# lyclyc52/Instance_NeRF

Measured on AMD Instinct MI355X. Metric: Msamples/sec (train+infer) 3D-FRONT 800x800 at 1/2/4/8 MI355X; PSNR parity, higher is better.
Workload: dtype f32; 1 GPU; render 800x800 synthetic 3D-FRONT-like room, hash-grid NeRF L=16 F=2 T=6119864 sigma+rgb (BASELINE configs[1]), one view per step per GPU; parallelism=views sharded over 1 GPU(s), no data-path collective

## Files before the change

### instance_nerf_amd/build.py

```python
import os
import shutil
import subprocess
import sys

HERE = os.path.dirname(os.path.abspath(__file__))
CSRC = os.path.join(HERE, "csrc")
LIB = os.path.join(CSRC, "libinr_hip.so")
SOURCES = ["raymarch.hip", "encoders.hip", "field_fused.hip", "roialign.hip"]
HEADERS = ["common.h", "grid_common.h", os.path.join("..", "..", "include", "inr.h")]
FLAGS = ["--offload-arch=gfx950", "-O3", "-std=c++17", "-fPIC", "-ffp-contract=off",
         "-munsafe-fp-atomics", "-Wall", "-Wno-unused-function"]


KERNEL_FILES = {
    "field": ["field_fused.hip", "common.h", "grid_common.h"],
    "scatter": ["encoders.hip", "common.h", "grid_common.h"],
}


def source_sha(kind=None):
    import hashlib
    h = hashlib.sha256()
    for f in sorted(KERNEL_FILES[kind] if kind else SOURCES + HEADERS):
        h.update(f.encode())
        h.update(open(os.path.join(CSRC, f), "rb").read())
    return h.hexdigest()


LIB_FP32 = os.path.join(CSRC, "libinr_hip_fp32.so")


def build_fp32(force=False, verbose=True):
    deps = [os.path.join(CSRC, f) for f in SOURCES + HEADERS] + [os.path.abspath(__file__)]
    if not force and os.path.exists(LIB_FP32) and all(os.path.getmtime(d) <= os.path.getmtime(LIB_FP32) for d in deps):
        return LIB_FP32
    hipcc = shutil.which("hipcc") or "/opt/rocm/bin/hipcc"
    objs = []
    for src in SOURCES:
        obj = os.path.join(CSRC, src.replace(".hip", ".fp32.o"))
        cmd = [hipcc, "-x", "hip", "-c", os.path.join(CSRC, src), "-o", obj, "-DINR_MLP_FP32=1"] + FLAGS
        if verbose:
            print(" ".join(cmd), flush=True)
        subprocess.check_call(cmd)
        objs.append(obj)
    subprocess.check_call([hipcc, "-shared", "-o", LIB_FP32] + objs + ["--offload-arch=gfx950"])
    return LIB_FP32


def _stale():
    if not os.path.exists(LIB):
        return True
    t = os.path.getmtime(LIB)
    deps = [os.path.join(CSRC, f) for f in SOURCES + HEADERS] + [os.path.abspath(__file__)]
    return any(os.path.getmtime(d) > t for d in deps)


def build(force=False, verbose=True):
    if not force and not _stale():
        return LIB
    hipcc = shutil.which("hipcc") or "/opt/rocm/bin/hipcc"
    if not os.path.exists(hipcc):
        raise RuntimeError("hipcc not found: cannot build libinr_hip.so")
    objs = []
    for src in SOURCES:
        obj = os.path.join(CSRC, src.replace(".hip", ".o"))
        cmd = [hipcc, "-x", "hip", "-c", os.path.join(CSRC, src), "-o", obj] + FLAGS
        if verbose:
            print(" ".join(cmd), flush=True)
        subprocess.check_call(cmd)
        objs.append(obj)
    cmd = [hipcc, "-shared", "-o", LIB] + objs + ["--offload-arch=gfx950"]
    if verbose:
        print(" ".join(cmd), flush=True)
    subprocess.check_call(cmd)
    return LIB


if __name__ == "__main__":
    build(force="--force" in sys.argv)
    build_fp32(force="--force" in sys.argv)
    print(LIB)
```

### instance_nerf_amd/csrc/field_fused.hip

```cpp
#include <atomic>
#include <mutex>
#include <type_traits>

#include "common.h"
#include "grid_common.h"

namespace inr {

typedef float f32x4 __attribute__((ext_vector_type(4)));
typedef __bf16 bf16x8 __attribute__((ext_vector_type(8)));

#ifndef INR_MLP_FP32
#define INR_MLP_FP32 0
#endif

#ifdef INR_PROBE_BUILD
#include "probe/field_probe.h"
#else
#if defined(INR_PROBE_MODE) || defined(INR_PROBE_STATIC) || defined(INR_PROBE_SLOW_XCD)
#error "INR_PROBE_* switches need -DINR_PROBE_BUILD (tools/build_probe.py): those variants produce wrong results"
#endif
#define INR_PROBE_PROLOGUE()
#define INR_PROBE_SCHEDULE(steal)
#define INR_PROBE_TILE()
#define INR_PROBE_AFTER_GATHER()
#define INR_PROBE_GEO_IS_OUTPUT 1
#define INR_PROBE_EPILOGUE()
#endif


constexpr int kSig0 = 0;
constexpr int kSig1 = kSig0 + 64 * 32;
constexpr int kCol0 = kSig1 + 16 * 64;
constexpr int kCol1 = kCol0 + 64 * 32;
constexpr int kCol2 = kCol1 + 64 * 64;
constexpr int kNerfFloats = kCol2 + 16 * 64;
constexpr int kIns0 = 0;
constexpr int kIns1 = kIns0 + 64 * 32;
constexpr int kIns2 = kIns1 + 64 * 64;

__host__ __device__ inline int frag_pos(int mt, int ks, int lane, int n_ks) {
  return ((mt * (n_ks / 4) + ks / 4) * 64 + lane) * 4 + (ks & 3);
}

__device__ __forceinline__ f32x4 mfma4(const float4 a, const f32x4 b, f32x4 c) {
  c = __builtin_amdgcn_mfma_f32_16x16x4f32(a.x, b[0], c, 0, 0, 0);
  c = __builtin_amdgcn_mfma_f32_16x16x4f32(a.y, b[1], c, 0, 0, 0);
  c = __builtin_amdgcn_mfma_f32_16x16x4f32(a.z, b[2], c, 0, 0, 0);
  c = __builtin_amdgcn_mfma_f32_16x16x4f32(a.w, b[3], c, 0, 0, 0);
  return c;
}
__device__ __forceinline__ float relu1(float x) { return __int_as_float(max(__float_as_int(x), 0)); }
__device__ __forceinline__ f32x4 relu4(f32x4 v) {
  v[0] = relu1(v[0]); v[1] = relu1(v[1]); v[2] = relu1(v[2]); v[3] = relu1(v[3]);
  return v;
}

struct LevelRec {
  uint4 a, b;
};
constexpr int kLevelRecBytes = 16 * sizeof(LevelRec);

__device__ __forceinline__ void stage_level_recs(const GridDesc& G, LevelRec* recs) {
  const int t = threadIdx.x;
  if (t < 16) {
    const int q = t >> 2, li = t & 3;
    const int l = (li >> 1) * 8 + 2 * q + (li & 1);
    const bool live = l < G.num_levels;
    const int lc = live ? l : 0;
    const uint32_t m = G.mask[lc], s = G.res1[lc];
    LevelRec r;
    r.a.x = live ? __float_as_uint(G.scales[lc]) : 0u;
    r.a.y = live ? G.offsets[lc] * 8u : 0u;
    r.a.z = !live ? 0u : (m ? 2654435761u : s);
    r.a.w = !live ? 0u : (m ? 805459861u : s * s);
    r.b.x = !live ? 0u : (m ? m : 0xFFFFFFFFu);
    r.b.y = (live && m) ? 1u : 0u;
    r.b.z = 0u; r.b.w = 0u;
    recs[t] = r;
  }
}

__device__ __forceinline__ bool slot_all_hashed(const GridDesc& G, int li) {
  bool ah = true;
#pragma unroll
  for (int qq = 0; qq < 4; ++qq) {
    const int lq = (li >> 1) * 8 + 2 * qq + (li & 1);
    ah = ah && (lq < G.num_levels) && (G.mask[lq < G.num_levels ? lq : 0] != 0);
  }
  return ah;
}

typedef unsigned int u32x2 __attribute__((__vector_size__(2 * sizeof(unsigned int))));

template <bool kHalf = false>
__device__ __forceinline__ u32x2 gather_row(__amdgpu_buffer_rsrc_t rsrc, uint32_t byte_off) {
  if constexpr (kHalf) {
    u32x2 r;
    r[0] = __builtin_amdgcn_raw_buffer_load_b32(rsrc, (int)(byte_off >> 1), 0, 0);
    r[1] = 0u;
    return r;
  } else {
    return __builtin_amdgcn_raw_buffer_load_b64(rsrc, (int)byte_off, 0, 0);
  }
}

typedef float f32x2 __attribute__((ext_vector_type(2)));

struct Gathered {
  u32x2 c[2][8];
  u32x2 f[4][4];
  float cfx[2], cfy[2], cfz[2];
  float fwx[4], ffy[4], ffz[4];
};

constexpr int kSliceLevels = 3;
constexpr int kWaitAfterCoarse = 8;
constexpr int kWaitBetweenFine = 4;
template <int N>
__device__ __forceinline__ void wait_vmcnt() {
  if constexpr (N >= 0) __builtin_amdgcn_s_waitcnt((N & 0xF) | (0x7 << 4) | (0xF << 8) | ((N >> 4) << 14));
}

template <bool kFineHashed, bool kHalf = false, bool kPre = false>
__device__ __forceinline__ void issue_gathers_impl(const LevelRec* __restrict__ my_recs, __amdgpu_buffer_rsrc_t rsrc,
                                                   float x0, float x1, float x2, Gathered& g) {
  const int q = (threadIdx.x >> 4) & 3;
  const uint32_t side = (uint32_t)(q & 1);
  const LevelRec* pair_recs = my_recs - 4 * (q & 1);
#pragma unroll
  for (int li = 0; li < 2; ++li) {
    const uint4 ra = my_recs[li].a;
    const float s = __uint_as_float(ra.x);
    const uint32_t base = ra.y, pa = ra.z, pb = ra.w;
    const uint32_t mask = my_recs[li].b.x;
    const float px = x0 * s + 0.5f, py = x1 * s + 0.5f, pz = x2 * s + 0.5f;
    g.cfx[li] = __builtin_amdgcn_fractf(px); g.cfy[li] = __builtin_amdgcn_fractf(py); g.cfz[li] = __builtin_amdgcn_fractf(pz);
    const uint32_t cx = (uint32_t)px, cy = (uint32_t)py, cz = (uint32_t)pz;
    const uint32_t hy0 = cy * pa, hy1 = hy0 + pa;
    const uint32_t hz0 = cz * pb, hz1 = hz0 + pb;
    const bool h = my_recs[li].b.y != 0;
    const uint32_t yz[4] = {h ? (hy0 ^ hz0) : (hy0 + hz0), h ? (hy1 ^ hz0) : (hy1 + hz0),
                            h ? (hy0 ^ hz1) : (hy0 + hz1), h ? (hy1 ^ hz1) : (hy1 + hz1)};
#pragma unroll
    for (int k = 0; k < 8; ++k) {
      const uint32_t c = cx + (k & 1);
      const uint32_t idx = (h ? (c ^ yz[k >> 1]) : (c + yz[k >> 1])) & mask;
      g.c[li][k] = gather_row<kHalf>(rsrc, base + idx * 8u);
    }
  }
#pragma unroll
  for (int i = 0; i < 4; ++i) {
    const LevelRec* rec = pair_recs + (i >> 1) * 4 + 2 + (i & 1);
    const uint4 ra = rec->a;
    const float s = __uint_as_float(ra.x);
    const uint32_t base = ra.y, pa = ra.z, pb = ra.w;
    const uint32_t mask = rec->b.x;
    const float px = x0 * s + 0.5f, py = x1 * s + 0.5f, pz = x2 * s + 0.5f;
    const float fx = __builtin_amdgcn_fractf(px);
    g.fwx[i] = side ? fx : 1.0f - fx;
    g.ffy[i] = __builtin_amdgcn_fractf(py); g.ffz[i] = __builtin_amdgcn_fractf(pz);
    const uint32_t c = (uint32_t)px + side, cy = (uint32_t)py, cz = (uint32_t)pz;
    const uint32_t hy0 = cy * pa, hy1 = hy0 + pa;
    const uint32_t hz0 = cz * pb, hz1 = hz0 + pb;
    if (i == 0) wait_vmcnt<kWaitAfterCoarse>();
    else wait_vmcnt<kWaitBetweenFine>();
    if constexpr (kPre) {
      const uint32_t keep = ((q >> 1) && i >= 4 - kSliceLevels) ? 0u : 0xFFFFFFFFu;
      g.f[i][0] = gather_row<kHalf>(rsrc, (base + ((c ^ (hy0 ^ hz0)) & mask) * 8u) & keep);
      g.f[i][1] = gather_row<kHalf>(rsrc, (base + ((c ^ (hy1 ^ hz0)) & mask) * 8u) & keep);
      g.f[i][2] = gather_row<kHalf>(rsrc, (base + ((c ^ (hy0 ^ hz1)) & mask) * 8u) & keep);
      g.f[i][3] = gather_row<kHalf>(rsrc, (base + ((c ^ (hy1 ^ hz1)) & mask) * 8u) & keep);
    } else if constexpr (kFineHashed) {
      g.f[i][0] = gather_row<kHalf>(rsrc, base + ((c ^ (hy0 ^ hz0)) & mask) * 8u);
      g.f[i][1] = gather_row<kHalf>(rsrc, base + ((c ^ (hy1 ^ hz0)) & mask) * 8u);
      g.f[i][2] = gather_row<kHalf>(rsrc, base + ((c ^ (hy0 ^ hz1)) & mask) * 8u);
      g.f[i][3] = gather_row<kHalf>(rsrc, base + ((c ^ (hy1 ^ hz1)) & mask) * 8u);
    } else {
      const bool h = rec->b.y != 0;
      const uint32_t yz[4] = {h ? (hy0 ^ hz0) : (hy0 + hz0), h ? (hy1 ^ hz0) : (hy1 + hz0),
                              h ? (hy0 ^ hz1) : (hy0 + hz1), h ? (hy1 ^ hz1) : (hy1 + hz1)};
#pragma unroll
      for (int k = 0; k < 4; ++k) {
        const uint32_t idx = (h ? (c ^ yz[k]) : (c + yz[k])) & mask;
        g.f[i][k] = gather_row<kHalf>(rsrc, base + idx * 8u);
      }
    }
  }
}

template <bool kHalf = false, bool kPre = false>
__device__ __forceinline__ void issue_gathers(const LevelRec* __restrict__ my_recs, const bool (&all_hashed)[4],
                                              __amdgpu_buffer_rsrc_t rsrc, float x0, float x1, float x2, Gathered& g) {
  if constexpr (kPre) issue_gathers_impl<true, kHalf, true>(my_recs, rsrc, x0, x1, x2, g);
  else if (all_hashed[2] && all_hashed[3]) issue_gathers_impl<true, kHalf>(my_recs, rsrc, x0, x1, x2, g);
  else issue_gathers_impl<false, kHalf>(my_recs, rsrc, x0, x1, x2, g);
}

template <bool kHalf = false>
__device__ __forceinline__ f32x2 row2(const u32x2 v) {
  const unsigned bx = v[0], by = v[1];
  if constexpr (kHalf) {
    typedef _Float16 h2 __attribute__((ext_vector_type(2)));
    const h2 h = __builtin_bit_cast(h2, bx);
    return f32x2{(float)h[0], (float)h[1]};
  } else {
    return f32x2{__uint_as_float(bx), __uint_as_float(by)};
  }
}

template <bool kHalf = false>
__device__ __forceinline__ void blend(const Gathered& g, f32x4& lo, f32x4& hi) {
#pragma unroll
  for (int li = 0; li < 2; ++li) {
    const f32x2 wx = {1.0f - g.cfx[li], g.cfx[li]};
    const float wy0 = 1.0f - g.cfy[li], wz0 = 1.0f - g.cfz[li];
    const f32x2 a = wx * wy0, b = wx * g.cfy[li];
    const f32x2 w[4] = {a * wz0, b * wz0, a * g.cfz[li], b * g.cfz[li]};
    f32x2 acc = {0.f, 0.f};
#pragma unroll
    for (int k = 0; k < 8; ++k) {
      const f32x2 wk = (k & 1) ? w[k >> 1].yy : w[k >> 1].xx;
      acc = __builtin_elementwise_fma(wk, row2<kHalf>(g.c[li][k]), acc);
    }
    lo[2 * li] = acc.x;
    lo[2 * li + 1] = acc.y;
  }
  f32x2 part[4];
#pragma unroll
  for (int i = 0; i < 4; ++i) {
    const f32x2 wy = {1.0f - g.ffy[i], g.ffy[i]};
    const f32x2 xy = wy * g.fwx[i];
    const f32x2 w0 = xy * (1.0f - g.ffz[i]), w1 = xy * g.ffz[i];
    f32x2 acc = {0.f, 0.f};
    acc = __builtin_elementwise_fma(w0.xx, row2<kHalf>(g.f[i][0]), acc);
    acc = __builtin_elementwise_fma(w0.yy, row2<kHalf>(g.f[i][1]), acc);
    acc = __builtin_elementwise_fma(w1.xx, row2<kHalf>(g.f[i][2]), acc);
    acc = __builtin_elementwise_fma(w1.yy, row2<kHalf>(g.f[i][3]), acc);
    part[i] = acc;
  }
#pragma unroll
  for (int t = 0; t < 4; ++t) {
    const int lv = t >> 1, ft = t & 1;
    const auto r = __builtin_amdgcn_permlane16_swap(__float_as_uint(part[lv][ft]), __float_as_uint(part[2 + lv][ft]), false, false);
    const unsigned r0 = r[0], r1 = r[1];
    hi[t] = __uint_as_float(r0) + __uint_as_float(r1);
  }
}


template <int N_MT, int N_G>
__device__ __forceinline__ void layer(const float4* __restrict__ w, int lane, const f32x4* in, f32x4* out) {
  if constexpr (N_MT == 1) {
    f32x4 a0 = {0.f, 0.f, 0.f, 0.f}, a1 = {0.f, 0.f, 0.f, 0.f};
#pragma unroll
    for (int g = 0; g < N_G; g += 2) {
      __builtin_amdgcn_sched_barrier(0);
      const float4 w0 = w[g * 64 + lane], w1 = w[(g + 1) * 64 + lane];
      a0 = __builtin_amdgcn_mfma_f32_16x16x4f32(w0.x, in[g][0], a0, 0, 0, 0);
      a1 = __builtin_amdgcn_mfma_f32_16x16x4f32(w1.x, in[g + 1][0], a1, 0, 0, 0);
      a0 = __builtin_amdgcn_mfma_f32_16x16x4f32(w0.y, in[g][1], a0, 0, 0, 0);
      a1 = __builtin_amdgcn_mfma_f32_16x16x4f32(w1.y, in[g + 1][1], a1, 0, 0, 0);
      a0 = __builtin_amdgcn_mfma_f32_16x16x4f32(w0.z, in[g][2], a0, 0, 0, 0);
      a1 = __builtin_amdgcn_mfma_f32_16x16x4f32(w1.z, in[g + 1][2], a1, 0, 0, 0);
      a0 = __builtin_amdgcn_mfma_f32_16x16x4f32(w0.w, in[g][3], a0, 0, 0, 0);
      a1 = __builtin_amdgcn_mfma_f32_16x16x4f32(w1.w, in[g + 1][3], a1, 0, 0, 0);
    }
    out[0] = a0 + a1;
  } else {
    f32x4 acc[N_MT];
#pragma unroll
    for (int mt = 0; mt < N_MT; ++mt) acc[mt] = f32x4{0.f, 0.f, 0.f, 0.f};
#pragma unroll
    for (int g = 0; g < N_G; ++g) {
      __builtin_amdgcn_sched_barrier(0);
      float4 wv[N_MT];
#pragma unroll
      for (int mt = 0; mt < N_MT; ++mt) wv[mt] = w[(mt * N_G + g) * 64 + lane];
#pragma unroll
      for (int mt = 0; mt < N_MT; ++mt) acc[mt] = __builtin_amdgcn_mfma_f32_16x16x4f32(wv[mt].x, in[g][0], acc[mt], 0, 0, 0);
#pragma unroll
      for (int mt = 0; mt < N_MT; ++mt) acc[mt] = __builtin_amdgcn_mfma_f32_16x16x4f32(wv[mt].y, in[g][1], acc[mt], 0, 0, 0);
#pragma unroll
      for (int mt = 0; mt < N_MT; ++mt) acc[mt] = __builtin_amdgcn_mfma_f32_16x16x4f32(wv[mt].z, in[g][2], acc[mt], 0, 0, 0);
#pragma unroll
      for (int mt = 0; mt < N_MT; ++mt) acc[mt] = __builtin_amdgcn_mfma_f32_16x16x4f32(wv[mt].w, in[g][3], acc[mt], 0, 0, 0);
    }
#pragma unroll
    for (int mt = 0; mt < N_MT; ++mt) out[mt] = acc[mt];
  }
}

struct SplitB {
  uint4 hi, lo;
};

__device__ __forceinline__ void split2(float x0, float x1, uint32_t& hi, uint32_t& lo) {
  const uint32_t u0 = __float_as_uint(x0), u1 = __float_as_uint(x1);
  hi = __builtin_amdgcn_perm(u1, u0, 0x07060302u);
  const float l0 = x0 - __uint_as_float(u0 & 0xFFFF0000u);
  const float l1 = x1 - __uint_as_float(u1 & 0xFFFF0000u);
  lo = __builtin_amdgcn_perm(__float_as_uint(l1), __float_as_uint(l0), 0x07060302u);
}
__device__ __forceinline__ SplitB split8(const f32x4 a, const f32x4 b) {
  SplitB r;
  split2(a[0], a[1], r.hi.x, r.lo.x);
  split2(a[2], a[3], r.hi.y, r.lo.y);
  split2(b[0], b[1], r.hi.z, r.lo.z);
  split2(b[2], b[3], r.hi.w, r.lo.w);
  return r;
}
__device__ __forceinline__ f32x4 mfma_bf(const uint4 a, const uint4 b, const f32x4 c) {
  return __builtin_amdgcn_mfma_f32_16x16x32_bf16(__builtin_bit_cast(bf16x8, a), __builtin_bit_cast(bf16x8, b), c, 0, 0, 0);
}

template <int N_MT, int N_S>
__device__ __forceinline__ void layer_bf(const uint4* __restrict__ w, int lane, const SplitB* in, f32x4* out) {
  if constexpr (N_MT == 1) {
    f32x4 a0 = {0.f, 0.f, 0.f, 0.f}, a1 = a0, a2 = a0;
#pragma unroll
    for (int st = 0; st < N_S; ++st) {
      __builtin_amdgcn_sched_barrier(0);
      const uint4 wh = w[(st * 2 + 0) * 64 + lane], wlo = w[(st * 2 + 1) * 64 + lane];
      a0 = mfma_bf(wh, in[st].hi, a0);
      a1 = mfma_bf(wlo, in[st].hi, a1);
      a2 = mfma_bf(wh, in[st].lo, a2);
    }
    out[0] = a0 + (a1 + a2);
  } else {
    f32x4 acc[N_MT];
#pragma unroll
    for (int mt = 0; mt < N_MT; ++mt) acc[mt] = f32x4{0.f, 0.f, 0.f, 0.f};
#pragma unroll
    for (int st = 0; st < N_S; ++st) {
      __builtin_amdgcn_sched_barrier(0);
      uint4 wh[N_MT], wlo[N_MT];
#pragma unroll
      for (int mt = 0; mt < N_MT; ++mt) {
        wh[mt] = w[((mt * N_S + st) * 2 + 0) * 64 + lane];
        wlo[mt] = w[((mt * N_S + st) * 2 + 1) * 64 + lane];
      }
#pragma unroll
      for (int mt = 0; mt < N_MT; ++mt) acc[mt] = mfma_bf(wh[mt], in[st].hi, acc[mt]);
#pragma unroll
      for (int mt = 0; mt < N_MT; ++mt) acc[mt] = mfma_bf(wlo[mt], in[st].hi, acc[mt]);
#pragma unroll
      for (int mt = 0; mt < N_MT; ++mt) acc[mt] = mfma_bf(wh[mt], in[st].lo, acc[mt]);
    }
#pragma unroll
    for (int mt = 0; mt < N_MT; ++mt) out[mt] = acc[mt];
  }
}

typedef _Float16 f16x8_t __attribute__((ext_vector_type(8)));
typedef _Float16 f16x2_t __attribute__((ext_vector_type(2)));
typedef float f32x2_t __attribute__((ext_vector_type(2)));
__device__ __forceinline__ uint32_t pack_f16x2(float a, float b) {
  const f32x2_t v = {a, b};
  return __builtin_bit_cast(uint32_t, __builtin_convertvector(v, f16x2_t));
}
template <int N_MT, int N_S>
__device__ __forceinline__ void layer_h1(const uint4* __restrict__ w, int lane, const uint4* in, f32x4* out) {
  f32x4 acc[N_MT];
#pragma unroll
  for (int mt = 0; mt < N_MT; ++mt) acc[mt] = f32x4{0.f, 0.f, 0.f, 0.f};
#pragma unroll
  for (int st = 0; st < N_S; ++st) {
    __builtin_amdgcn_sched_barrier(0);
#pragma unroll
    for (int mt = 0; mt < N_MT; ++mt)
      acc[mt] = __builtin_amdgcn_mfma_f32_16x16x32_f16(__builtin_bit_cast(f16x8_t, w[((mt * N_S + st) * 2 + 0) * 64 + lane]),
                                                       __builtin_bit_cast(f16x8_t, in[st]), acc[mt], 0, 0, 0);
  }
#pragma unroll
  for (int mt = 0; mt < N_MT; ++mt) out[mt] = acc[mt];
}

template <int N_MT, int N_G, bool kFast = false>
__device__ __forceinline__ void mlp_layer(const float4* __restrict__ wsec, int lane, const f32x4* in, f32x4* out) {
#if INR_MLP_FP32
  layer<N_MT, N_G>(wsec, lane, in, out);
#else
  if constexpr (kFast) {
    uint4 b[N_G / 2];
#pragma unroll
    for (int st = 0; st < N_G / 2; ++st)
      b[st] = uint4{pack_f16x2(in[2 * st][0], in[2 * st][1]), pack_f16x2(in[2 * st][2], in[2 * st][3]),
                    pack_f16x2(in[2 * st + 1][0], in[2 * st + 1][1]), pack_f16x2(in[2 * st + 1][2], in[2 * st + 1][3])};
    layer_h1<N_MT, N_G / 2>(reinterpret_cast<const uint4*>(wsec), lane, b, out);
  } else {
    SplitB b[N_G / 2];
#pragma unroll
    for (int st = 0; st < N_G / 2; ++st) b[st] = split8(in[2 * st], in[2 * st + 1]);
    layer_bf<N_MT, N_G / 2>(reinterpret_cast<const uint4*>(wsec), lane, b, out);
  }
#endif
}

__device__ __forceinline__ float select4(int q, float a, float b, float c, float d) {
  return q == 0 ? a : (q == 1 ? b : (q == 2 ? c : d));
}

struct TileIn {
  float x0, x1, x2;
  float d0, d1, d2;
  bool oob;
};

__device__ __forceinline__ float to_x01(float x, float bound, float rb, float) { return (x + bound) / rb; }

template <bool kDir>
__device__ __forceinline__ void load_tile_in(const float* __restrict__ x, const float* __restrict__ d, int64_t m,
                                             float bound, float rb, float rb_inv, TileIn& t) {
  t.x0 = to_x01(x[m * 3 + 0], bound, rb, rb_inv);
  t.x1 = to_x01(x[m * 3 + 1], bound, rb, rb_inv);
  t.x2 = to_x01(x[m * 3 + 2], bound, rb, rb_inv);
  t.oob = oob01(t.x0, t.x1, t.x2);
  if (t.oob) t.x0 = t.x1 = t.x2 = 0.0f;
  if constexpr (kDir) {
    t.d0 = d[m * 3]; t.d1 = d[m * 3 + 1]; t.d2 = d[m * 3 + 2];
  }
}

constexpr int kXcdChunkLog2 = 10;
#ifndef INR_STEAL_SHIFT
#define INR_STEAL_SHIFT 1
#endif
constexpr int kStealRoundsShift = INR_STEAL_SHIFT;
struct TileSched {
  int64_t lo, hi;
  int64_t first;
  int64_t stride;
  int64_t main_local = 0, tail_base = 0;
  int64_t n_main = 0, tail = 0;
  int64_t static_local = 0;
  uint32_t xcd = 0;
  bool interleaved = false, hybrid = false;
  __device__ __forceinline__ int64_t tile_of(int y, int64_t u) const {
    if (u < main_local) return ((((u >> kXcdChunkLog2) << 3) + y) << kXcdChunkLog2) + (u & ((1 << kXcdChunkLog2) - 1));
    return n_main + tail * y / 8 + (u - main_local);
  }
  __device__ __forceinline__ int64_t local_end(int y) const { return main_local + tail * (y + 1) / 8 - tail * y / 8; }
  __device__ __forceinline__ int64_t tile(int64_t i) const {
    if (interleaved) {
      const int64_t u = first + i * stride;
      if (u < main_local)
        return ((((u >> kXcdChunkLog2) << 3) + xcd) << kXcdChunkLog2) + (u & ((1 << kXcdChunkLog2) - 1));
      return tail_base + (u - main_local);
    }
    return first + i * stride;
  }
};
__device__ __forceinline__ TileSched make_sched(int64_t n_tiles, int waves_per_block, bool steal = false) {
  const int nb = gridDim.x, b = blockIdx.x;
  const int w = threadIdx.x >> 6;
  TileSched s;
  if (nb % 8 == 0) {
    const int xcd = b & 7, local = b >> 3, per = nb >> 3;
    const int64_t rounds = n_tiles >> (kXcdChunkLog2 + 3);
    if (rounds >= 4) {
      const int64_t n_main = rounds << (kXcdChunkLog2 + 3), tail = n_tiles - n_main;
      s.interleaved = true;
      s.xcd = (uint32_t)xcd;
      s.main_local = rounds << kXcdChunkLog2;
      s.n_main = n_main;
      s.tail = tail;
      s.hybrid = steal;
      s.static_local = steal ? (rounds - max((int64_t)1, rounds >> kStealRoundsShift)) << kXcdChunkLog2 : s.main_local;
      s.tail_base = n_main + tail * xcd / 8;
      s.lo = 0;
      s.hi = n_main + tail * (xcd + 1) / 8;
      s.first = (int64_t)local * waves_per_block + w;
      s.stride = (int64_t)per * waves_per_block;
      return s;
    }
    s.lo = n_tiles * xcd / 8;
    s.hi = n_tiles * (xcd + 1) / 8;
    s.first = s.lo + (int64_t)local * waves_per_block + w;
    s.stride = (int64_t)per * waves_per_block;
  } else {
    s.lo = 0;
    s.hi = n_tiles;
    s.first = (int64_t)b * waves_per_block + w;
    s.stride = (int64_t)nb * waves_per_block;
  }
  return s;
}

constexpr int kFieldThreads = 512;
constexpr int kGroupChunkLog2 = 6;
constexpr int kGroupDraw = 1;
constexpr int kGroupPools = 4;
struct GroupDraw {
  unsigned long long* cursor;
  int owner, n_owner;
  __device__ __forceinline__ void init(unsigned long long* cursors, int pools) {
    const int n_xcd = (gridDim.x % 8 == 0) ? 8 : 1;
    const int n_pool = (gridDim.x % (8 * pools) == 0) ? pools : 1;
    const int xcd = (n_xcd == 8) ? (int)(blockIdx.x & 7) : 0;
    const int pool = (n_pool > 1) ? (int)((blockIdx.x >> 3) % pools) : 0;
    owner = pool * n_xcd + xcd;
    n_owner = n_pool * n_xcd;
    cursor = cursors + owner;
  }
  __device__ __forceinline__ int64_t group_of(uint32_t u) const {
    const int64_t chunk = (int64_t)(u >> kGroupChunkLog2) * n_owner + owner;
    return (chunk << kGroupChunkLog2) + (u & ((1u << kGroupChunkLog2) - 1u));
  }
  __device__ __forceinline__ int64_t draw() const { return group_of((uint32_t)atomicAdd(cursor, (unsigned long long)kGroupDraw)); }
};
constexpr int kStealPools = 4, kStealOwners = 8 * kStealPools, kStealDraw = 4, kStealBlockLog2 = 6;
struct TileWalk {
  TileSched s;
  unsigned long long* cur;
  int lane, own, owner, sub;
  int64_t it, k_base;
  unsigned long long raw_next;
  bool dyn;
  __device__ __forceinline__ void init(const TileSched& sched, unsigned long long* cursors) {
    s = sched; cur = cursors; lane = threadIdx.x & 63; it = 0; dyn = false; sub = kStealDraw; k_base = 0; raw_next = 0;
    own = owner = (int)(((blockIdx.x >> 3) % kStealPools) * 8 + (blockIdx.x & 7));
    if (!cursors) s.hybrid = false;
    if (!s.hybrid) s.static_local = s.main_local;
  }
  __device__ __forceinline__ int64_t pool_len(int o) const {
    const int64_t nb = (s.local_end(o & 7) - s.static_local + (1 << kStealBlockLog2) - 1) >> kStealBlockLog2;
    const int p = o >> 3;
    return nb > p ? ((nb - p + kStealPools - 1) / kStealPools) << kStealBlockLog2 : 0;
  }
  __device__ __forceinline__ int64_t local_of(int o, int64_t k) const {
    return s.static_local + ((((k >> kStealBlockLog2) * kStealPools) + (o >> 3)) << kStealBlockLog2) +
           (k & ((1 << kStealBlockLog2) - 1));
  }
  __device__ __forceinline__ unsigned long long issue(int o) const {
    unsigned long long v = 0;
    if (lane == 0) v = atomicAdd(cur + o, (unsigned long long)kStealDraw);
    return v;
  }
  __device__ __forceinline__ static int64_t uniform(unsigned long long v) {
    return (int64_t)(((unsigned long long)(uint32_t)__builtin_amdgcn_readfirstlane((int)(v >> 32)) << 32) |
                     (uint32_t)__builtin_amdgcn_readfirstlane((int)v));
  }
  __device__ __forceinline__ int scan() const {
    bool live = false;
    if (lane < kStealOwners) live = (int64_t)__hip_atomic_load(cur + lane, __ATOMIC_RELAXED, __HIP_MEMORY_SCOPE_AGENT) < pool_len(lane);
    const uint32_t mask = (uint32_t)__ballot(live);
    for (int i = 0; i < kStealOwners; ++i) {
      const int o = (((own >> 3) + i) % kStealPools) * 8 + (((own & 7) + i / kStealPools) & 7);
      if ((mask >> o) & 1u) return o;
    }
    return -1;
  }
  __device__ __forceinline__ int64_t next() {
    if (!dyn) {
      if (!s.hybrid) {
        const int64_t t = s.tile(it++);
        return t < s.hi ? t : -1;
      }
      const int64_t u = s.first + (it++) * s.stride;
      if (u < s.static_local) return s.tile_of((int)s.xcd, u);
      dyn = true;
      raw_next = issue(owner);
    }
    for (;;) {
      if (sub < kStealDraw) {
        const int64_t u = local_of(owner, k_base + sub);
        ++sub;
        if (u < s.local_end(owner & 7)) return s.tile_of(owner & 7, u);
        continue;
      }
      int64_t k = uniform(raw_next);
      while (k >= pool_len(owner)) {
        const int o = scan();
        if (o < 0) return -1;
        owner = o;
        k = uniform(issue(owner));
      }
      k_base = k;
      sub = 0;
      raw_next = issue(owner);
    }
  }
};
constexpr int kFieldMinWaves = 2;

__device__ __forceinline__ f32x4 load4(const float* p) {
  const float4 v = *reinterpret_cast<const float4*>(p);
  return f32x4{v.x, v.y, v.z, v.w};
}
__device__ __forceinline__ void store4(float* p, f32x4 v) {
  *reinterpret_cast<float4*>(p) = make_float4(v[0], v[1], v[2], v[3]);
}
__device__ __forceinline__ f32x4 mask4(f32x4 g, f32x4 h) {
  return f32x4{h[0] > 0.f ? g[0] : 0.f, h[1] > 0.f ? g[1] : 0.f, h[2] > 0.f ? g[2] : 0.f, h[3] > 0.f ? g[3] : 0.f};
}

struct NerfSave {
  float *enc, *h1, *so, *cin, *c1, *c2;
};

template <bool kColor, bool kTable = false, int kSave = 0, bool kHalf = false, bool kFast = false, bool kPre = false>
__global__ void __launch_bounds__(kFieldThreads, kFieldMinWaves) k_nerf_fwd(const float* __restrict__ x, const float* __restrict__ d,
                                                               int64_t M, const int32_t* __restrict__ n_dev, float bound,
                                                               const float2* __restrict__ emb, uint32_t emb_bytes, GridDesc G,
                                                               const float4* __restrict__ packed, float density_scale,
                                                               float* __restrict__ sigma, float* __restrict__ rgb,
                                                               float* __restrict__ geo, const int32_t* __restrict__ ray_ids,
                                                               const float4* __restrict__ shq, NerfSave sv,
                                                               unsigned long long* __restrict__ steal) {
  extern __shared__ __attribute__((aligned(16))) float4 wl[];
  INR_PROBE_PROLOGUE();
  __builtin_amdgcn_s_setprio(3);
  constexpr int kStage = (kColor ? kNerfFloats : kCol0) / 4;
  for (int i = threadIdx.x; i < kStage; i += kFieldThreads) wl[i] = packed[i];
  LevelRec* recs = reinterpret_cast<LevelRec*>(wl + kStage);
  stage_level_recs(G, recs);
  __syncthreads();

  constexpr int kWaves = kFieldThreads / 64;
  const int lane = threadIdx.x & 63, q = lane >> 4, j = lane & 15;
  int64_t n = M;
  if (n_dev) n = min((int64_t)*n_dev, M);
  const int64_t n_tiles = (n + 15) >> 4;
  const float rb = 2.0f * bound;
  const float rb_inv = 0.0f;
  INR_PROBE_SCHEDULE(steal);
  TileWalk walk;
  walk.init(make_sched(n_tiles, kWaves, steal != nullptr), steal);

  const bool all_hashed[4] = {slot_all_hashed(G, 0), slot_all_hashed(G, 1), slot_all_hashed(G, 2), slot_all_hashed(G, 3)};
  const __amdgpu_buffer_rsrc_t rsrc = __builtin_amdgcn_make_buffer_rsrc((void*)emb, 0, (int)emb_bytes, 0x00020000);

  for (int64_t tile = walk.next(); tile >= 0; tile = walk.next()) {
    INR_PROBE_TILE();
    const int64_t m = tile * 16 + j;
    const bool valid = m < n;
    TileIn me;
    f32x4 sh_in = {0.f, 0.f, 0.f, 0.f};
    if constexpr (kTable) {
      const int64_t mm = valid ? m : n - 1;
      me.x0 = x[mm * 3 + 0]; me.x1 = x[mm * 3 + 1]; me.x2 = x[mm * 3 + 2];
      const float4 t4 = shq[(int64_t)ray_ids[mm] * 4 + q];
      sh_in = f32x4{t4.x, t4.y, t4.z, t4.w};
    } else {
      load_tile_in<kColor>(x, d, valid ? m : n - 1, bound, rb, rb_inv, me);
    }

    f32x4 enc[2];
    {
      Gathered g;
      uint32_t rec_off = (uint32_t)q * 4u * (uint32_t)sizeof(LevelRec);
      asm volatile("" : "+v"(rec_off));
      typedef float v2f __attribute__((ext_vector_type(2)));
      v2f fine_a = {0.f, 0.f}, fine_b = {0.f, 0.f};
      if constexpr (kPre) {
        static_assert(!kPre || kTable, "the sliced feed is a variant of the table feed");
        static_assert(kSliceLevels == 3, "lane map below");
        const v2f* pre = reinterpret_cast<const v2f*>(d);
        const int64_t m_pad = (M + 31) & ~(int64_t)31, mm = valid ? m : n - 1;
        const int sl = (q & 1) ? 1 : 0;
        fine_a = __builtin_nontemporal_load(pre + (int64_t)sl * m_pad + mm);
        fine_b = __builtin_nontemporal_load(pre + (int64_t)(sl + 1) * m_pad + mm);
      }
      issue_gathers<kHalf, kPre>(reinterpret_cast<const LevelRec*>(reinterpret_cast<const char*>(recs) + rec_off), all_hashed,
                                 rsrc, me.x0, me.x1, me.x2, g);
      __builtin_amdgcn_sched_barrier(0);
      blend<kHalf>(g, enc[0], enc[1]);
      if constexpr (kPre) {
        if (q == 2) enc[1] = f32x4{enc[1][0], enc[1][1], fine_a.x, fine_a.y};
        else if (q == 3) enc[1] = f32x4{fine_a.x, fine_a.y, fine_b.x, fine_b.y};
      }
    }
    if constexpr (!kTable) {
      if (me.oob) enc[0] = enc[1] = f32x4{0.f, 0.f, 0.f, 0.f};
    }
    INR_PROBE_AFTER_GATHER();

    f32x4 h1[4];
    mlp_layer<4, 2, kFast>(wl + kSig0 / 4, lane, enc, h1);
#pragma unroll
    for (int t = 0; t < 4; ++t) h1[t] = relu4(h1[t]);
    f32x4 h2[1];
    mlp_layer<1, 4, kFast>(wl + kSig1 / 4, lane, h1, h2);

    if (valid) {
      if (q == 0) sigma[m] = __expf(h2[0][0]) * density_scale;
      if (INR_PROBE_GEO_IS_OUTPUT && geo) {
#pragma unroll
        for (int r = 0; r < 4; ++r) {
          const int row = 4 * q + r;
          if (row >= 1) geo[m * 15 + row - 1] = h2[0][r];
        }
      }
    }

    if constexpr (kColor) {
      f32x4 cin[2];
      if constexpr (kTable) {
        cin[0] = sh_in;
      } else {
        float sh[16];
        sh4(me.d0, me.d1, me.d2, sh);
#pragma unroll
        for (int ks = 0; ks < 4; ++ks) cin[0][ks] = select4(q, sh[4 * ks], sh[4 * ks + 1], sh[4 * ks + 2], sh[4 * ks + 3]);
      }
      cin[1] = h2[0];
      f32x4 c1[4], c2[4], o[1];
      mlp_layer<4, 2, kFast>(wl + kCol0 / 4, lane, cin, c1);
#pragma unroll
      for (int t = 0; t < 4; ++t) c1[t] = relu4(c1[t]);
      mlp_layer<4, 4, kFast>(wl + kCol1 / 4, lane, c1, c2);
#pragma unroll
      for (int t = 0; t < 4; ++t) c2[t] = relu4(c2[t]);
      mlp_layer<1, 4, kFast>(wl + kCol2 / 4, lane, c2, o);
      if constexpr (kSave == 2) {
        if (valid) {
#pragma unroll
          for (int t = 0; t < 2; ++t) store4(sv.enc + m * 32 + 16 * t + 4 * q, enc[t]);
        }
      }
      if constexpr (kSave == 1) {
        if (valid) {
#pragma unroll
          for (int t = 0; t < 2; ++t) store4(sv.enc + m * 32 + 16 * t + 4 * q, enc[t]);
          store4(sv.so + m * 16 + 4 * q, h2[0]);
#pragma unroll
          for (int t = 0; t < 4; ++t) {
            store4(sv.h1 + m * 64 + 16 * t + 4 * q, h1[t]);
            store4(sv.c1 + m * 64 + 16 * t + 4 * q, c1[t]);
            store4(sv.c2 + m * 64 + 16 * t + 4 * q, c2[t]);
          }
#pragma unroll
          for (int ks = 0; ks < 4; ++ks) sv.cin[m * 32 + 4 * ks + q] = cin[0][ks];
#pragma unroll
          for (int r = 0; r < 4; ++r) {
            const int row = 4 * q + r;
            sv.cin[m * 32 + (row >= 1 ? 15 + row : 31)] = row >= 1 ? h2[0][r] : 0.f;
          }
        }
      }
      if (valid && q == 0) {
        rgb[m * 3 + 0] = __frcp_rn(1.0f + __expf(-o[0][0]));
        rgb[m * 3 + 1] = __frcp_rn(1.0f + __expf(-o[0][1]));
        rgb[m * 3 + 2] = __frcp_rn(1.0f + __expf(-o[0][2]));
      }
    }
  }
  INR_PROBE_EPILOGUE();
}

constexpr int kSliceThreads = 256;
constexpr int kSliceTilesPerIter = 4;
struct SliceX {
  float x0, x1, x2;
};
__device__ __forceinline__ SliceX slice_load_x(const float* __restrict__ x01, int64_t m, int64_t M) {
  const int64_t mm = m < M ? m : M - 1;
  const float* p = x01 + mm * 3;
  return SliceX{__builtin_nontemporal_load(p), __builtin_nontemporal_load(p + 1), __builtin_nontemporal_load(p + 2)};
}
__global__ void __launch_bounds__(kSliceThreads) k_grid_fine_slices(const float* __restrict__ x01, int64_t M,
                                                                    const float2* __restrict__ emb, uint32_t emb_bytes,
                                                                    GridDesc G, float* __restrict__ pre) {
  const int slice = blockIdx.y;
  const int l = 16 - kSliceLevels + slice;
  const float sc = G.scales[l];
  const uint32_t m_ = G.mask[l], res1 = G.res1[l];
  const bool h = m_ != 0;
  const uint32_t base = G.offsets[l] * 8u, pa = h ? 2654435761u : res1, pb = h ? 805459861u : res1 * res1;
  const uint32_t mask = h ? m_ : 0xFFFFFFFFu;
  const __amdgpu_buffer_rsrc_t rsrc = __builtin_amdgcn_make_buffer_rsrc((void*)emb, 0, (int)emb_bytes, 0x00020000);
  const int lane = threadIdx.x & 63, w = threadIdx.x >> 6;
  const uint32_t side = (uint32_t)(lane & 1);
  constexpr int kWaves = kSliceThreads / 64;
  constexpr int kT = kSliceTilesPerIter;
  const int64_t m_pad = (M + 31) & ~(int64_t)31;
  const int64_t n_iter = (M + 32 * kT - 1) / (32 * kT);
  float* __restrict__ out = pre + (int64_t)slice * m_pad * 2;
  for (int64_t it = (int64_t)blockIdx.x * kWaves + w; it < n_iter; it += (int64_t)gridDim.x * kWaves) {
    u32x2 rows[kT][4];
    float wx[kT], fy[kT], fz[kT];
#pragma unroll
    for (int t = 0; t < kT; ++t) {
      const SliceX X = slice_load_x(x01, (it * kT + t) * 32 + (lane >> 1), M);
      const float px = X.x0 * sc + 0.5f, py = X.x1 * sc + 0.5f, pz = X.x2 * sc + 0.5f;
      const float fx = __builtin_amdgcn_fractf(px);
      wx[t] = side ? fx : 1.0f - fx;
      fy[t] = __builtin_amdgcn_fractf(py); fz[t] = __builtin_amdgcn_fractf(pz);
      const uint32_t c = (uint32_t)px + side, cy = (uint32_t)py, cz = (uint32_t)pz;
      const uint32_t hy0 = cy * pa, hy1 = hy0 + pa;
      const uint32_t hz0 = cz * pb, hz1 = hz0 + pb;
      const uint32_t yz[4] = {h ? (hy0 ^ hz0) : (hy0 + hz0), h ? (hy1 ^ hz0) : (hy1 + hz0),
                              h ? (hy0 ^ hz1) : (hy0 + hz1), h ? (hy1 ^ hz1) : (hy1 + hz1)};
#pragma unroll
      for (int k = 0; k < 4; ++k) {
        const uint32_t idx = (h ? (c ^ yz[k]) : (c + yz[k])) & mask;
        rows[t][k] = gather_row<false>(rsrc, base + idx * 8u);
      }
    }
#pragma unroll
    for (int t = 0; t < kT; ++t) {
      const f32x2 wy = {1.0f - fy[t], fy[t]};
      const f32x2 xy = wy * wx[t];
      const f32x2 w0 = xy * (1.0f - fz[t]), w1 = xy * fz[t];
      f32x2 acc = {0.f, 0.f};
      acc = __builtin_elementwise_fma(w0.xx, row2<false>(rows[t][0]), acc);
      acc = __builtin_elementwise_fma(w0.yy, row2<false>(rows[t][1]), acc);
      acc = __builtin_elementwise_fma(w1.xx, row2<false>(rows[t][2]), acc);
      acc = __builtin_elementwise_fma(w1.yy, row2<false>(rows[t][3]), acc);
      const float ox = __shfl_xor(acc.x, 1), oy = __shfl_xor(acc.y, 1);
      const float v = side ? acc.y + oy : acc.x + ox;
      const int64_t m = (it * kT + t) * 32 + (lane >> 1);
      if (m < M) __builtin_nontemporal_store(v, out + m * 2 + side);
    }
  }
}

struct LatticeDesc {
  const float* ax_w;
  const float* ax_l;
  const float* ax_h;
  int W, L, H, Wp;
};
constexpr int kMaxExtractDirs = 8;
template <bool kLattice>
__global__ void __launch_bounds__(kFieldThreads, kFieldMinWaves) k_nerf_fwd_dirs(
    const float* __restrict__ x, int64_t M, float bound, const float2* __restrict__ emb, uint32_t emb_bytes, GridDesc G,
    const float4* __restrict__ packed, const float* __restrict__ sh_dirs , int D, float4* __restrict__ out,
    LatticeDesc lat, float logit_min) {
  extern __shared__ __attribute__((aligned(16))) float4 wl[];
  constexpr int kStage = kNerfFloats / 4;
  for (int i = threadIdx.x; i < kStage; i += kFieldThreads) wl[i] = packed[i];
  LevelRec* recs = reinterpret_cast<LevelRec*>(wl + kStage);
  stage_level_recs(G, recs);
  float* shl = reinterpret_cast<float*>(recs + 16);
  for (int i = threadIdx.x; i < D * 16; i += kFieldThreads) {
    const int d = i >> 4, qq = (i >> 2) & 3, ks = i & 3;
    shl[i] = sh_dirs[d * 16 + 4 * ks + qq];
  }
  __syncthreads();
  constexpr int kWaves = kFieldThreads / 64;
  const int lane = threadIdx.x & 63, q = lane >> 4, j = lane & 15;
  const int64_t n_tiles = (M + 15) >> 4;
  const float rb = 2.0f * bound;
  const TileSched sched = make_sched(n_tiles, kWaves);
  const bool all_hashed[4] = {slot_all_hashed(G, 0), slot_all_hashed(G, 1), slot_all_hashed(G, 2), slot_all_hashed(G, 3)};
  const __amdgpu_buffer_rsrc_t rsrc = __builtin_amdgcn_make_buffer_rsrc((void*)emb, 0, (int)emb_bytes, 0x00020000);
  const float inv_d = 1.0f / (float)D;
  for (int64_t it = 0, tile = sched.tile(0); tile < sched.hi; tile = sched.tile(++it)) {
    int64_t m = tile * 16 + j;
    bool valid = m < M;
    TileIn me;
    if constexpr (kLattice) {
      const int64_t row = m / lat.Wp;
      const int iw = (int)(m - row * lat.Wp);
      const int il = (int)(row / lat.H), ih = (int)(row - (int64_t)il * lat.H);
      valid = valid && iw < lat.W;
      const int cw = min(iw, lat.W - 1), cl = min(il, lat.L - 1);
      me.x0 = to_x01(fminf(fmaxf(lat.ax_w[cw], -bound), bound), bound, rb, 0.0f);
      me.x1 = to_x01(fminf(fmaxf(lat.ax_l[cl], -bound), bound), bound, rb, 0.0f);
      me.x2 = to_x01(fminf(fmaxf(lat.ax_h[ih], -bound), bound), bound, rb, 0.0f);
      me.oob = oob01(me.x0, me.x1, me.x2);
      if (me.oob) me.x0 = me.x1 = me.x2 = 0.0f;
      m = ((int64_t)cw * lat.L + cl) * lat.H + ih;
    } else {
      load_tile_in<false>(x, nullptr, valid ? m : M - 1, bound, rb, 0.0f, me);
    }
    f32x4 enc[2];
    {
      Gathered g;
      uint32_t rec_off = (uint32_t)q * 4u * (uint32_t)sizeof(LevelRec);
      asm volatile("" : "+v"(rec_off));
      issue_gathers(reinterpret_cast<const LevelRec*>(reinterpret_cast<const char*>(recs) + rec_off), all_hashed, rsrc,
                    me.x0, me.x1, me.x2, g);
      __builtin_amdgcn_sched_barrier(0);
      blend(g, enc[0], enc[1]);
    }
    if (me.oob) enc[0] = enc[1] = f32x4{0.f, 0.f, 0.f, 0.f};
    f32x4 h1[4], h2[1];
    mlp_layer<4, 2>(wl + kSig0 / 4, lane, enc, h1);
#pragma unroll
    for (int t = 0; t < 4; ++t) h1[t] = relu4(h1[t]);
    mlp_layer<1, 4>(wl + kSig1 / 4, lane, h1, h2);
    float r = 0.f, g = 0.f, b = 0.f;
    for (int d = 0; d < D; ++d) {
      f32x4 cin[2], c1[4], c2[4], o[1];
      const float4 s4 = *reinterpret_cast<const float4*>(shl + d * 16 + q * 4);
      cin[0] = f32x4{s4.x, s4.y, s4.z, s4.w};
      cin[1] = h2[0];
      mlp_layer<4, 2>(wl + kCol0 / 4, lane, cin, c1);
#pragma unroll
      for (int t = 0; t < 4; ++t) c1[t] = relu4(c1[t]);
      mlp_layer<4, 4>(wl + kCol1 / 4, lane, c1, c2);
#pragma unroll
      for (int t = 0; t < 4; ++t) c2[t] = relu4(c2[t]);
      mlp_layer<1, 4>(wl + kCol2 / 4, lane, c2, o);
      r += __frcp_rn(1.0f + __expf(-o[0][0]));
      g += __frcp_rn(1.0f + __expf(-o[0][1]));
      b += __frcp_rn(1.0f + __expf(-o[0][2]));
    }
    if (valid && q == 0) out[m] = make_float4(r * inv_d, g * inv_d, b * inv_d, fmaxf(h2[0][0], logit_min));
  }
}

template <int K_MT, int kSave = 0>
__global__ void __launch_bounds__(kFieldThreads, kFieldMinWaves) k_instance_fwd(const float* __restrict__ x, int64_t M,
                                                                   const int32_t* __restrict__ n_dev, float bound,
                                                                   const float2* __restrict__ emb, uint32_t emb_bytes,
                                                                   GridDesc G, const float4* __restrict__ packed,
                                                                   float* __restrict__ logits, float* __restrict__ enc_out,
                                                                   float* __restrict__ h1_out, float* __restrict__ h2_out) {
  extern __shared__ __attribute__((aligned(16))) float4 wl[];
  constexpr int K = K_MT * 16;
  constexpr int kStage = (kIns2 + K * 64) / 4;
  for (int i = threadIdx.x; i < kStage; i += kFieldThreads) wl[i] = packed[i];
  LevelRec* recs = reinterpret_cast<LevelRec*>(wl + kStage);
  stage_level_recs(G, recs);
  __syncthreads();

  constexpr int kWaves = kFieldThreads / 64;
  const int lane = threadIdx.x & 63, q = lane >> 4, j = lane & 15;
  int64_t n = M;
  if (n_dev) n = min((int64_t)*n_dev, M);
  const int64_t n_tiles = (n + 15) >> 4;
  const float rb = 2.0f * bound;
  const float rb_inv = 0.0f;
  const TileSched sched = make_sched(n_tiles, kWaves);

  const bool all_hashed[4] = {slot_all_hashed(G, 0), slot_all_hashed(G, 1), slot_all_hashed(G, 2), slot_all_hashed(G, 3)};
  const __amdgpu_buffer_rsrc_t rsrc = __builtin_amdgcn_make_buffer_rsrc((void*)emb, 0, (int)emb_bytes, 0x00020000);

  for (int64_t it = 0, tile = sched.tile(0); tile < sched.hi; tile = sched.tile(++it)) {
    const int64_t m = tile * 16 + j;
    const bool valid = m < n;
    TileIn me;
    load_tile_in<false>(x, nullptr, valid ? m : n - 1, bound, rb, rb_inv, me);
    f32x4 enc[2];
    {
      Gathered g;
      uint32_t rec_off = (uint32_t)q * 4u * (uint32_t)sizeof(LevelRec);
      asm volatile("" : "+v"(rec_off));
      issue_gathers(reinterpret_cast<const LevelRec*>(reinterpret_cast<const char*>(recs) + rec_off), all_hashed, rsrc,
                    me.x0, me.x1, me.x2, g);
      __builtin_amdgcn_sched_barrier(0);
      blend(g, enc[0], enc[1]);
    }
    if (me.oob) enc[0] = enc[1] = f32x4{0.f, 0.f, 0.f, 0.f};
    f32x4 h1[4], h2[4], o[K_MT];
    mlp_layer<4, 2>(wl + kIns0 / 4, lane, enc, h1);
#pragma unroll
    for (int t = 0; t < 4; ++t) h1[t] = relu4(h1[t]);
    mlp_layer<4, 4>(wl + kIns1 / 4, lane, h1, h2);
#pragma unroll
    for (int t = 0; t < 4; ++t) h2[t] = relu4(h2[t]);
    mlp_layer<K_MT, 4>(wl + kIns2 / 4, lane, h2, o);
    if (valid) {
#pragma unroll
      for (int mt = 0; mt < K_MT; ++mt) {
        float4 v = make_float4(o[mt][0], o[mt][1], o[mt][2], o[mt][3]);
        *reinterpret_cast<float4*>(logits + m * K + 16 * mt + 4 * q) = v;
      }
      if constexpr (kSave != 0) {
#pragma unroll
        for (int t = 0; t < 2; ++t)
          *reinterpret_cast<float4*>(enc_out + m * 32 + 16 * t + 4 * q) = make_float4(enc[t][0], enc[t][1], enc[t][2], enc[t][3]);
      }
      if constexpr (kSave == 1) {
#pragma unroll
        for (int t = 0; t < 4; ++t) {
          *reinterpret_cast<float4*>(h1_out + m * 64 + 16 * t + 4 * q) = make_float4(h1[t][0], h1[t][1], h1[t][2], h1[t][3]);
          *reinterpret_cast<float4*>(h2_out + m * 64 + 16 * t + 4 * q) = make_float4(h2[t][0], h2[t][1], h2[t][2], h2[t][3]);
        }
      }
    }
  }
}

constexpr uint8_t kLabelEmpty = 255;
constexpr int kNoChannel = 0x7fffffff;
template <int K_MT>
__global__ void __launch_bounds__(kFieldThreads, kFieldMinWaves) k_instance_lattice(
    LatticeDesc lat, float bound, const float2* __restrict__ emb_n, uint32_t emb_n_bytes, GridDesc Gn,
    const float4* __restrict__ packed_n, float density_scale, float sigma_thresh, const float2* __restrict__ emb_i,
    uint32_t emb_i_bytes, GridDesc Gi, const float4* __restrict__ packed_i, int K, uint8_t* __restrict__ labels,
    float* __restrict__ confidence, float* __restrict__ logit_out) {
  extern __shared__ __attribute__((aligned(16))) float4 wl[];
  constexpr int kStageN = kCol0 / 4;
  constexpr int kStageI = (kIns2 + K_MT * 16 * 64) / 4;
  const float4* wn = wl;
  const float4* wi = wl + kStageN;
  for (int i = threadIdx.x; i < kStageN; i += kFieldThreads) wl[i] = packed_n[i];
  for (int i = threadIdx.x; i < kStageI; i += kFieldThreads) wl[kStageN + i] = packed_i[i];
  LevelRec* recs_n = reinterpret_cast<LevelRec*>(wl + kStageN + kStageI);
  LevelRec* recs_i = recs_n + 16;
  stage_level_recs(Gn, recs_n);
  stage_level_recs(Gi, recs_i);
  __syncthreads();

  constexpr int kWaves = kFieldThreads / 64;
  const int lane = threadIdx.x & 63, q = lane >> 4, j = lane & 15;
  const int64_t n_tiles = ((int64_t)lat.Wp * lat.L * lat.H) >> 4;
  const float rb = 2.0f * bound;
  const TileSched sched = make_sched(n_tiles, kWaves);
  const bool hashed_n[4] = {slot_all_hashed(Gn, 0), slot_all_hashed(Gn, 1), slot_all_hashed(Gn, 2), slot_all_hashed(Gn, 3)};
  const bool hashed_i[4] = {slot_all_hashed(Gi, 0), slot_all_hashed(Gi, 1), slot_all_hashed(Gi, 2), slot_all_hashed(Gi, 3)};
  const __amdgpu_buffer_rsrc_t rsrc_n = __builtin_amdgcn_make_buffer_rsrc((void*)emb_n, 0, (int)emb_n_bytes, 0x00020000);
  const __amdgpu_buffer_rsrc_t rsrc_i = __builtin_amdgcn_make_buffer_rsrc((void*)emb_i, 0, (int)emb_i_bytes, 0x00020000);
  for (int64_t it = 0, tile = sched.tile(0); tile < sched.hi; tile = sched.tile(++it)) {
    const int64_t m = tile * 16 + j;
    const int64_t row = m / lat.Wp;
    const int iw = (int)(m - row * lat.Wp);
    const int il = (int)(row / lat.H), ih = (int)(row - (int64_t)il * lat.H);
    const bool valid = iw < lat.W;
    const int cw = min(iw, lat.W - 1);
    TileIn me;
    me.x0 = to_x01(fminf(fmaxf(lat.ax_w[cw], -bound), bound), bound, rb, 0.0f);
    me.x1 = to_x01(fminf(fmaxf(lat.ax_l[il], -bound), bound), bound, rb, 0.0f);
// ... 1818 lines not shown
```

Before: 6474 Msamples/s.

## Software-pipeline split-bf16 MLP layers with interleaved weight prefetch and ReLU splitting

Replaces the per-layer split-bf16 MFMA MLP calls in the sigma and color nets with hand-scheduled chains. These prefetch the next weight fragment one slot ahead and do the ReLU plus hi/lo bf16 split of the previous output tile inside the current tile's MFMA slot, using sched_group_barrier to interleave MFMA and VALU work. The aim is to hide weight-load latency and layer-boundary VALU work behind matrix instructions. The cost is higher register pressure, which may lower occupancy, and more rigid instruction scheduling. The shared split2 helper moves into a new header.

```diff
diff --git a/instance_nerf_amd/build.py b/instance_nerf_amd/build.py
--- a/instance_nerf_amd/build.py
+++ b/instance_nerf_amd/build.py
@@ -7,13 +7,13 @@
 CSRC = os.path.join(HERE, "csrc")
 LIB = os.path.join(CSRC, "libinr_hip.so")
 SOURCES = ["raymarch.hip", "encoders.hip", "field_fused.hip", "roialign.hip"]
-HEADERS = ["common.h", "grid_common.h", os.path.join("..", "..", "include", "inr.h")]
+HEADERS = ["common.h", "grid_common.h", "bf16_split.h", os.path.join("..", "..", "include", "inr.h")]
 FLAGS = ["--offload-arch=gfx950", "-O3", "-std=c++17", "-fPIC", "-ffp-contract=off",
          "-munsafe-fp-atomics", "-Wall", "-Wno-unused-function"]
 
 
 KERNEL_FILES = {
-    "field": ["field_fused.hip", "common.h", "grid_common.h"],
+    "field": ["field_fused.hip", "common.h", "grid_common.h", "bf16_split.h"],
     "scatter": ["encoders.hip", "common.h", "grid_common.h"],
 }
 
diff --git a/instance_nerf_amd/csrc/bf16_split.h b/instance_nerf_amd/csrc/bf16_split.h
--- /dev/null
+++ b/instance_nerf_amd/csrc/bf16_split.h
@@ -0,0 +1,15 @@
+#pragma once
+#include <hip/hip_runtime.h>
+#include <stdint.h>
+
+namespace inr {
+
+__device__ __forceinline__ void split2(float x0, float x1, uint32_t& hi, uint32_t& lo) {
+  const uint32_t u0 = __float_as_uint(x0), u1 = __float_as_uint(x1);
+  hi = __builtin_amdgcn_perm(u1, u0, 0x07060302u);
+  const float l0 = x0 - __uint_as_float(u0 & 0xFFFF0000u);
+  const float l1 = x1 - __uint_as_float(u1 & 0xFFFF0000u);
+  lo = __builtin_amdgcn_perm(__float_as_uint(l1), __float_as_uint(l0), 0x07060302u);
+}
+
+}
diff --git a/instance_nerf_amd/csrc/field_fused.hip b/instance_nerf_amd/csrc/field_fused.hip
--- a/instance_nerf_amd/csrc/field_fused.hip
+++ b/instance_nerf_amd/csrc/field_fused.hip
@@ -2,6 +2,7 @@
 #include <mutex>
 #include <type_traits>
 
+#include "bf16_split.h"
 #include "common.h"
 #include "grid_common.h"
 
@@ -295,13 +296,6 @@
   uint4 hi, lo;
 };
 
-__device__ __forceinline__ void split2(float x0, float x1, uint32_t& hi, uint32_t& lo) {
-  const uint32_t u0 = __float_as_uint(x0), u1 = __float_as_uint(x1);
-  hi = __builtin_amdgcn_perm(u1, u0, 0x07060302u);
-  const float l0 = x0 - __uint_as_float(u0 & 0xFFFF0000u);
-  const float l1 = x1 - __uint_as_float(u1 & 0xFFFF0000u);
-  lo = __builtin_amdgcn_perm(__float_as_uint(l1), __float_as_uint(l0), 0x07060302u);
-}
 __device__ __forceinline__ SplitB split8(const f32x4 a, const f32x4 b) {
   SplitB r;
   split2(a[0], a[1], r.hi.x, r.lo.x);
@@ -395,6 +389,122 @@
     layer_bf<N_MT, N_G / 2>(reinterpret_cast<const uint4*>(wsec), lane, b, out);
   }
 #endif
+}
+
+struct WFrag {
+  uint4 h, l;
+};
+__device__ __forceinline__ WFrag load_w(const uint4* __restrict__ w, int frag, int lane) {
+  return WFrag{w[(frag * 2 + 0) * 64 + lane], w[(frag * 2 + 1) * 64 + lane]};
+}
+template <class Fill>
+__device__ __forceinline__ void mfma_slot(f32x4& a0, f32x4& a1, f32x4& a2, const WFrag wf, const SplitB& b, Fill&& fill) {
+  a0 = mfma_bf(wf.h, b.hi, a0);
+  a1 = mfma_bf(wf.l, b.hi, a1);
+  a2 = mfma_bf(wf.h, b.lo, a2);
+  fill();
+#pragma unroll
+  for (int i = 0; i < 3; ++i) {
+    __builtin_amdgcn_sched_group_barrier(0x8, 1, 0);
+    __builtin_amdgcn_sched_group_barrier(0x2, 4, 0);
+  }
+  __builtin_amdgcn_sched_barrier(0);
+}
+__device__ __forceinline__ void relu_split_tile(f32x4& v, SplitB* b, int t) {
+  v = relu4(v);
+  uint32_t h0, l0, h1, l1;
+  split2(v[0], v[1], h0, l0);
+  split2(v[2], v[3], h1, l1);
+  SplitB& d = b[t >> 1];
+  if (t & 1) { d.hi.z = h0; d.hi.w = h1; d.lo.z = l0; d.lo.w = l1; }
+  else { d.hi.x = h0; d.hi.y = h1; d.lo.x = l0; d.lo.y = l1; }
+}
+template <int N_S, class Fill>
+__device__ __forceinline__ void layer_bf_tiles(const uint4* __restrict__ w, int lane, WFrag wf, const SplitB* in, f32x4* out,
+                                               Fill&& fill) {
+  f32x4 acc[4];
+#pragma unroll
+  for (int mt = 0; mt < 4; ++mt) acc[mt] = f32x4{0.f, 0.f, 0.f, 0.f};
+#pragma unroll
+  for (int st = 0; st < N_S; ++st) {
+#pragma unroll
+    for (int mt = 0; mt < 4; ++mt) {
+      const int nx = st * 4 + mt + 1;
+      const WFrag cur = wf;
+      if (nx < 4 * N_S) wf = load_w(w, (nx & 3) * N_S + (nx >> 2), lane);
+      mfma_slot(acc[mt], acc[mt], acc[mt], cur, in[st], [&] { fill(st, mt); });
+      if (st == N_S - 1) out[mt] = acc[mt];
+    }
+  }
+}
+template <int N_S, class Fill>
+__device__ __forceinline__ void layer_bf_one(const uint4* __restrict__ w, int lane, WFrag wf, const SplitB* in, f32x4* out,
+                                             Fill&& fill) {
+  f32x4 a0 = {0.f, 0.f, 0.f, 0.f}, a1 = a0, a2 = a0;
+#pragma unroll
+  for (int st = 0; st < N_S; ++st) {
+    const WFrag cur = wf;
+    if (st + 1 < N_S) wf = load_w(w, st + 1, lane);
+    mfma_slot(a0, a1, a2, cur, in[st], [&] { fill(st); });
+  }
+  out[0] = a0 + (a1 + a2);
+}
+
+template <bool kFast = false>
+__device__ __forceinline__ void sigma_net(const float4* __restrict__ wl, int lane, const f32x4* enc, f32x4* h1, f32x4* h2) {
+  if constexpr (INR_MLP_FP32 || kFast) {
+    mlp_layer<4, 2, kFast>(wl + kSig0 / 4, lane, enc, h1);
+#pragma unroll
+    for (int t = 0; t < 4; ++t) h1[t] = relu4(h1[t]);
+    mlp_layer<1, 4, kFast>(wl + kSig1 / 4, lane, h1, h2);
+  } else {
+    const uint4* w0 = reinterpret_cast<const uint4*>(wl + kSig0 / 4);
+    const uint4* w1 = reinterpret_cast<const uint4*>(wl + kSig1 / 4);
+    WFrag wf1 = load_w(w0, 0, lane);
+    const WFrag wf0 = wf1;
+    const SplitB be = split8(enc[0], enc[1]);
+    SplitB bh[2];
+    layer_bf_tiles<1>(w0, lane, wf0, &be, h1, [&](int, int mt) {
+      if (mt > 0) relu_split_tile(h1[mt - 1], bh, mt - 1);
+      if (mt == 3) wf1 = load_w(w1, 0, lane);
+    });
+    layer_bf_one<2>(w1, lane, wf1, bh, h2, [&](int st) {
+      if (st == 0) relu_split_tile(h1[3], bh, 3);
+    });
+  }
+}
+template <bool kFast = false>
+__device__ __forceinline__ void color_net(const float4* __restrict__ wl, int lane, const f32x4* cin, f32x4* c1, f32x4* c2,
+                                          f32x4* o) {
+  if constexpr (INR_MLP_FP32 || kFast) {
+    mlp_layer<4, 2, kFast>(wl + kCol0 / 4, lane, cin, c1);
+#pragma unroll
+    for (int t = 0; t < 4; ++t) c1[t] = relu4(c1[t]);
+    mlp_layer<4, 4, kFast>(wl + kCol1 / 4, lane, c1, c2);
+#pragma unroll
+    for (int t = 0; t < 4; ++t) c2[t] = relu4(c2[t]);
+    mlp_layer<1, 4, kFast>(wl + kCol2 / 4, lane, c2, o);
+  } else {
+    const uint4* w0 = reinterpret_cast<const uint4*>(wl + kCol0 / 4);
+    const uint4* w1 = reinterpret_cast<const uint4*>(wl + kCol1 / 4);
+    const uint4* w2 = reinterpret_cast<const uint4*>(wl + kCol2 / 4);
+    WFrag wf1 = load_w(w0, 0, lane), wf2 = wf1;
+    const WFrag wf0 = wf1;
+    const SplitB bc = split8(cin[0], cin[1]);
+    SplitB b1[2], b2[2];
+    layer_bf_tiles<1>(w0, lane, wf0, &bc, c1, [&](int, int mt) {
+      if (mt > 0) relu_split_tile(c1[mt - 1], b1, mt - 1);
+      if (mt == 3) wf1 = load_w(w1, 0, lane);
+    });
+    layer_bf_tiles<2>(w1, lane, wf1, b1, c2, [&](int st, int mt) {
+      if (st == 0 && mt == 0) relu_split_tile(c1[3], b1, 3);
+      if (st == 1 && mt > 0) relu_split_tile(c2[mt - 1], b2, mt - 1);
+      if (st == 1 && mt == 3) wf2 = load_w(w2, 0, lane);
+    });
+    layer_bf_one<2>(w2, lane, wf2, b2, o, [&](int st) {
+      if (st == 0) relu_split_tile(c2[3], b2, 3);
+    });
+  }
 }
 
 __device__ __forceinline__ float select4(int q, float a, float b, float c, float d) {
@@ -676,12 +786,8 @@
     }
     INR_PROBE_AFTER_GATHER();
 
-    f32x4 h1[4];
-    mlp_layer<4, 2, kFast>(wl + kSig0 / 4, lane, enc, h1);
-#pragma unroll
-    for (int t = 0; t < 4; ++t) h1[t] = relu4(h1[t]);
-    f32x4 h2[1];
-    mlp_layer<1, 4, kFast>(wl + kSig1 / 4, lane, h1, h2);
+    f32x4 h1[4], h2[1];
+    sigma_net<kFast>(wl, lane, enc, h1, h2);
 
     if (valid) {
       if (q == 0) sigma[m] = __expf(h2[0][0]) * density_scale;
@@ -706,13 +812,7 @@
       }
       cin[1] = h2[0];
       f32x4 c1[4], c2[4], o[1];
-      mlp_layer<4, 2, kFast>(wl + kCol0 / 4, lane, cin, c1);
-#pragma unroll
-      for (int t = 0; t < 4; ++t) c1[t] = relu4(c1[t]);
-      mlp_layer<4, 4, kFast>(wl + kCol1 / 4, lane, c1, c2);
-#pragma unroll
-      for (int t = 0; t < 4; ++t) c2[t] = relu4(c2[t]);
-      mlp_layer<1, 4, kFast>(wl + kCol2 / 4, lane, c2, o);
+      color_net<kFast>(wl, lane, cin, c1, c2, o);
       if constexpr (kSave == 2) {
         if (valid) {
 #pragma unroll
```

Measured after the change: 6516 Msamples/s (median of 6 runs). No clear change (+0.7%).
